# toverainc/willow-inference-server

Measured on NVIDIA H100. Metric: Whisper large-v2 realtime multiple (audio s / s), beam 5, 3.84 s utterance, higher is better.
Workload: dtype f16

## Files before the change

willow_inference_server_b200/csrc/encoder.cu:

```cuda
#include <algorithm>
#include <mutex>

#include "kernels.h"
#include "ptx.cuh"

namespace wisb {

void make_tmap_f16_2d(CUtensorMap* map, const void* ptr, long long cols, long long rows, long long ld, int box_cols,
                      int box_rows);

namespace {

constexpr int C1_FT = 64;
constexpr int C1_CT = 64;
template <int NM>
constexpr int c1_smem_bytes() { return (NM * (C1_FT + 2) + 3 * NM * (C1_CT + 1)) * 4; }

template <int NM>
__global__ void __launch_bounds__(256)
conv1_gelu_kernel(const float* __restrict__ mel, const __half* __restrict__ w, const float* __restrict__ bias,
                  __half* __restrict__ h1, int d) {
  constexpr int C1_K = 3 * NM;
  extern __shared__ float c1_smem[];
  float (*xm)[C1_FT + 2] = reinterpret_cast<float (*)[C1_FT + 2]>(c1_smem);
  float (*wt)[C1_CT + 1] = reinterpret_cast<float (*)[C1_CT + 1]>(c1_smem + NM * (C1_FT + 2));
  const int b = blockIdx.z;
  const int f0 = blockIdx.x * C1_FT;
  const int c0 = blockIdx.y * C1_CT;
  const int tid = threadIdx.x;
  const float* melb = mel + static_cast<long long>(b) * NM * N_FRAMES;
  for (int i = tid; i < NM * (C1_FT + 2); i += 256) {
    const int ci = i / (C1_FT + 2), fl = i % (C1_FT + 2);
    const int f = f0 + fl - 1;
    xm[ci][fl] = (f >= 0 && f < N_FRAMES) ? melb[ci * N_FRAMES + f] : 0.f;
  }
  for (int i = tid; i < C1_CT * C1_K; i += 256) {
    const int co = i / C1_K, kk = i % C1_K;
    wt[kk][co] = __half2float(w[static_cast<long long>(c0 + co) * C1_K + kk]);
  }
  __syncthreads();
  const int tc = tid % 16;
  const int tf = tid / 16;
  float acc[4][4];
#pragma unroll
  for (int i = 0; i < 4; ++i)
#pragma unroll
    for (int j = 0; j < 4; ++j) acc[i][j] = 0.f;
  for (int kk = 0; kk < C1_K; ++kk) {
    const int k = kk / NM, ci = kk - k * NM;
    float a[4], bb[4];
#pragma unroll
    for (int i = 0; i < 4; ++i) a[i] = xm[ci][tf * 4 + i + k];
#pragma unroll
    for (int j = 0; j < 4; ++j) bb[j] = wt[kk][tc * 4 + j];
#pragma unroll
    for (int i = 0; i < 4; ++i)
#pragma unroll
      for (int j = 0; j < 4; ++j) acc[i][j] = fmaf(a[i], bb[j], acc[i][j]);
  }
#pragma unroll
  for (int i = 0; i < 4; ++i) {
    const int f = f0 + tf * 4 + i;
    if (f >= N_FRAMES) continue;
    __half* o = h1 + (static_cast<long long>(b) * H1_ROWS + 1 + f) * d + c0 + tc * 4;
    __half2 v0 = __floats2half2_rn(gelu_erf(acc[i][0] + bias[c0 + tc * 4 + 0]), gelu_erf(acc[i][1] + bias[c0 + tc * 4 + 1]));
    __half2 v1 = __floats2half2_rn(gelu_erf(acc[i][2] + bias[c0 + tc * 4 + 2]), gelu_erf(acc[i][3] + bias[c0 + tc * 4 + 3]));
    uint2 u;
    u.x = *reinterpret_cast<uint32_t*>(&v0);
    u.y = *reinterpret_cast<uint32_t*>(&v1);
    *reinterpret_cast<uint2*>(o) = u;
  }
}

constexpr int LN_MAX_IT = 12;

__global__ void __launch_bounds__(256)
layernorm_f32_to_f16_kernel(const float* __restrict__ x, const float* __restrict__ g, const float* __restrict__ b,
                            __half* __restrict__ y, int rows, int d) {
  pdl_launch_dependents();
  pdl_wait();
  const int row = blockIdx.x * 8 + (threadIdx.x >> 5);
  const int lane = threadIdx.x & 31;
  if (row >= rows) return;
  const int iters = d / 128;
  const float4* xr = reinterpret_cast<const float4*>(x + static_cast<long long>(row) * d);
  float4 v[LN_MAX_IT];
  float s = 0.f;
#pragma unroll
  for (int i = 0; i < LN_MAX_IT; ++i)
    if (i < iters) {
      v[i] = xr[i * 32 + lane];
      s += v[i].x + v[i].y + v[i].z + v[i].w;
    }
  const float mean = warp_sum(s) / d;
  float q = 0.f;
#pragma unroll
  for (int i = 0; i < LN_MAX_IT; ++i)
    if (i < iters) {
      const float a0 = v[i].x - mean, a1 = v[i].y - mean, a2 = v[i].z - mean, a3 = v[i].w - mean;
      q += a0 * a0 + a1 * a1 + a2 * a2 + a3 * a3;
    }
  const float rstd = rsqrtf(warp_sum(q) / d + 1e-5f);
  const float4* g4 = reinterpret_cast<const float4*>(g);
  const float4* b4 = reinterpret_cast<const float4*>(b);
  uint2* yr = reinterpret_cast<uint2*>(y + static_cast<long long>(row) * d);
#pragma unroll
  for (int i = 0; i < LN_MAX_IT; ++i)
    if (i < iters) {
      const float4 gg = __ldg(g4 + i * 32 + lane), bb = __ldg(b4 + i * 32 + lane);
      __half2 h0 = __floats2half2_rn((v[i].x - mean) * rstd * gg.x + bb.x, (v[i].y - mean) * rstd * gg.y + bb.y);
      __half2 h1 = __floats2half2_rn((v[i].z - mean) * rstd * gg.z + bb.z, (v[i].w - mean) * rstd * gg.w + bb.w);
      uint2 u;
      u.x = *reinterpret_cast<uint32_t*>(&h0);
      u.y = *reinterpret_cast<uint32_t*>(&h1);
      yr[i * 32 + lane] = u;
    }
}

constexpr int AT_THREADS = 128;
constexpr int AT_BM = 64, AT_BN = 128;
constexpr int AT_NB = T_ENC_PAD / AT_BN;
constexpr int AT_TILE = 128 * 64 * 2;
constexpr int AT_Q_BYTES = AT_BM * 64 * 2;
constexpr int AT_SMEM = AT_Q_BYTES + 4 * AT_TILE  + 64  + 1024 ;

__device__ __forceinline__ uint32_t pack_half2(float a, float b) {
  __half2 h = __floats2half2_rn(a, b);
  return *reinterpret_cast<uint32_t*>(&h);
}

template <bool kVMN>
__global__ void __launch_bounds__(AT_THREADS, 3)
enc_attn_kernel(const __grid_constant__ CUtensorMap map_q, const __grid_constant__ CUtensorMap map_k,
                const __grid_constant__ CUtensorMap map_v, __half* __restrict__ ctx, int d, int H) {
  extern __shared__ uint8_t at_raw[];
  const uint32_t raw_addr = smem_u32(at_raw);
  const uint32_t base = (raw_addr + 1023u) & ~1023u;
  const uint32_t sQ = base;
  const uint32_t sK = base + AT_Q_BYTES;
  const uint32_t sV = sK + 2 * AT_TILE;
  const uint32_t bar0 = sV + 2 * AT_TILE;
  const uint32_t q_full = bar0;
  auto kv_full = [&](int s) { return bar0 + 8u * (1 + s); };

  const int tid = threadIdx.x, warp = tid >> 5, lane = tid & 31;
  const int qt = blockIdx.x, h = blockIdx.y, b = blockIdx.z;
  const int row0 = b * T_ENC_PAD + qt * AT_BM;

  if (tid == 0) {
    mbar_init(q_full, 1);
    mbar_init(kv_full(0), 1);
    mbar_init(kv_full(1), 1);
    fence_mbar_init();
    tma_prefetch_desc(&map_q);
    tma_prefetch_desc(&map_k);
    tma_prefetch_desc(&map_v);
  }
  __syncthreads();
  pdl_launch_dependents();
  pdl_wait();

  auto load_kv = [&](int j) {
    const int st = j & 1;
    mbar_arrive_expect_tx(kv_full(st), 2 * AT_TILE);
    tma_load_2d(sK + st * AT_TILE, &map_k, kv_full(st), d + h * HEAD_DIM, b * T_ENC_PAD + j * AT_BN);
    if (kVMN) {
      tma_load_2d(sV + st * AT_TILE, &map_v, kv_full(st), 2 * d + h * HEAD_DIM, b * T_ENC_PAD + j * AT_BN);
    } else {
      tma_load_2d(sV + st * AT_TILE, &map_v, kv_full(st), j * AT_BN, (b * H + h) * HEAD_DIM);
      tma_load_2d(sV + st * AT_TILE + AT_TILE / 2, &map_v, kv_full(st), j * AT_BN + 64, (b * H + h) * HEAD_DIM);
    }
  };
  if (tid == 0) {
    mbar_arrive_expect_tx(q_full, AT_Q_BYTES);
    tma_load_2d(sQ, &map_q, q_full, h * HEAD_DIM, row0);
    load_kv(0);
    load_kv(1);
  }

  const int cq = 2 * (lane & 3);
  const float c = 0.125f * 1.4426950408889634f;
  float m_run[2] = {-INFINITY, -INFINITY}, l_run[2] = {0.f, 0.f};
  float o[HEAD_DIM / 2];
#pragma unroll
  for (int i = 0; i < HEAD_DIM / 2; ++i) o[i] = 0.f;
  const uint64_t dq = make_desc_sw128(sQ, 1024);
  mbar_wait(q_full, 0);
#pragma unroll 1
  for (int j = 0; j < AT_NB; ++j) {
    const int st = j & 1;
    mbar_wait(kv_full(st), (j >> 1) & 1u);
    float s[AT_BN / 2];
    const uint64_t dk = make_desc_sw128(sK + st * AT_TILE, 1024);
    wgmma_fence();
#pragma unroll
    for (int k = 0; k < 4; ++k) wgmma_ss<AT_BN, 0, 0>(s, dq + 2u * k, dk + 2u * k, k != 0 ? 1u : 0u);
    wgmma_commit();
    wgmma_wait<0>();
    wgmma_reg_fence(s);
    const int kv0 = j * AT_BN;
    if (kv0 + AT_BN > T_ENC) {
#pragma unroll
      for (int i = 0; i < AT_BN / 2; ++i)
        if (kv0 + (i >> 2) * 8 + cq + (i & 1) >= T_ENC) s[i] = -INFINITY;
    }
    float alpha[2], mc[2];
#pragma unroll
    for (int hr = 0; hr < 2; ++hr) {
      float mx = -INFINITY;
#pragma unroll
      for (int nb = 0; nb < AT_BN / 8; ++nb) mx = fmaxf(mx, fmaxf(s[4 * nb + 2 * hr], s[4 * nb + 2 * hr + 1]));
      mx = fmaxf(mx, __shfl_xor_sync(0xffffffffu, mx, 1));
      mx = fmaxf(mx, __shfl_xor_sync(0xffffffffu, mx, 2));
      const float m_new = fmaxf(m_run[hr], mx);
      alpha[hr] = exp2f((m_run[hr] - m_new) * c);
      mc[hr] = m_new * c;
      m_run[hr] = m_new;
    }
    uint32_t pa[AT_BN / 16][4];
    float rs[2] = {0.f, 0.f};
#pragma unroll
    for (int kk = 0; kk < AT_BN / 16; ++kk) {
      float p[8];
#pragma unroll
      for (int i = 0; i < 8; ++i) {
        p[i] = exp2f(fmaf(s[8 * kk + i], c, -mc[(i >> 1) & 1]));
        rs[(i >> 1) & 1] += p[i];
      }
      pa[kk][0] = pack_half2(p[0], p[1]);
      pa[kk][1] = pack_half2(p[2], p[3]);
      pa[kk][2] = pack_half2(p[4], p[5]);
      pa[kk][3] = pack_half2(p[6], p[7]);
    }
#pragma unroll
    for (int hr = 0; hr < 2; ++hr) l_run[hr] = l_run[hr] * alpha[hr] + rs[hr];
#pragma unroll
    for (int i = 0; i < HEAD_DIM / 2; ++i) o[i] *= alpha[(i >> 1) & 1];
    wgmma_fence();
#pragma unroll
    for (int kk = 0; kk < AT_BN / 16; ++kk) {
      uint64_t dv;
      if (kVMN)
        dv = make_desc_sw128(sV + st * AT_TILE + kk * 2048, 1024);
      else
        dv = make_desc_sw128(sV + st * AT_TILE + (kk >> 2) * (AT_TILE / 2), 1024) + 2u * (kk & 3);
      wgmma_rs<HEAD_DIM, kVMN ? 1 : 0>(o, pa[kk], dv, 1u);
    }
    wgmma_commit();
    wgmma_wait<0>();
    wgmma_reg_fence(o);
    __syncthreads();
    if (tid == 0 && j + 2 < AT_NB) load_kv(j + 2);
  }
#pragma unroll
  for (int hr = 0; hr < 2; ++hr) {
    l_run[hr] += __shfl_xor_sync(0xffffffffu, l_run[hr], 1);
    l_run[hr] += __shfl_xor_sync(0xffffffffu, l_run[hr], 2);
  }
  const float inv[2] = {1.0f / l_run[0], 1.0f / l_run[1]};
#pragma unroll
  for (int hr = 0; hr < 2; ++hr) {
    const int r = warp * 16 + (lane >> 2) + 8 * hr;
    __half* out = ctx + static_cast<long long>(row0 + r) * d + h * HEAD_DIM + cq;
#pragma unroll
    for (int nb = 0; nb < HEAD_DIM / 8; ++nb)
      *reinterpret_cast<uint32_t*>(out + nb * 8) = pack_half2(o[4 * nb + 2 * hr] * inv[hr], o[4 * nb + 2 * hr + 1] * inv[hr]);
  }
}

__global__ void __launch_bounds__(128)
enc_attn_ref_kernel(const __half* __restrict__ qkv, __half* __restrict__ ctx, int d) {
  const int b = blockIdx.z, h = blockIdx.y;
  const int t = blockIdx.x * 128 + threadIdx.x;
  const long long ld = 3LL * d;
  const __half* base = qkv + static_cast<long long>(b) * T_ENC_PAD * ld;
  float q[HEAD_DIM], acc[HEAD_DIM];
  for (int e = 0; e < HEAD_DIM; ++e) {
    q[e] = __half2float(base[t * ld + h * HEAD_DIM + e]);
    acc[e] = 0.f;
  }
  float m = -INFINITY, l = 0.f;
  for (int k = 0; k < T_ENC; ++k) {
    const __half* kr = base + k * ld + d + h * HEAD_DIM;
    float s = 0.f;
    for (int e = 0; e < HEAD_DIM; ++e) s = fmaf(q[e], __half2float(kr[e]), s);
    s *= 0.125f;
    const float mn = fmaxf(m, s);
    const float a = __expf(m - mn), p = __expf(s - mn);
    const __half* vr = base + k * ld + 2 * d + h * HEAD_DIM;
    for (int e = 0; e < HEAD_DIM; ++e) acc[e] = acc[e] * a + p * __half2float(vr[e]);
    l = l * a + p;
    m = mn;
  }
  __half* o = ctx + (static_cast<long long>(b) * T_ENC_PAD + t) * d + h * HEAD_DIM;
  for (int e = 0; e < HEAD_DIM; ++e) o[e] = __float2half_rn(acc[e] / l);
}

}

void conv1_gelu_run(const float* mel, const __half* w, const float* bias, __half* h1, int B, int d, int n_mels,
                    cudaStream_t stream) {
  WISB_REQUIRE(d % C1_CT == 0, "conv1: d_model must be a multiple of 64");
  WISB_REQUIRE(n_mels == 80 || n_mels == 128, "conv1: n_mels must be 80 or 128");
  static std::atomic<unsigned long long> once{0};
  once_per_device(once, [] {
    WISB_CUDA(cudaFuncSetAttribute(conv1_gelu_kernel<80>, cudaFuncAttributeMaxDynamicSharedMemorySize, c1_smem_bytes<80>()));
    WISB_CUDA(cudaFuncSetAttribute(conv1_gelu_kernel<128>, cudaFuncAttributeMaxDynamicSharedMemorySize, c1_smem_bytes<128>()));
  });
  dim3 grid(cdiv(N_FRAMES, C1_FT), d / C1_CT, B);
  if (n_mels == 80)
    conv1_gelu_kernel<80><<<grid, 256, c1_smem_bytes<80>(), stream>>>(mel, w, bias, h1, d);
  else
    conv1_gelu_kernel<128><<<grid, 256, c1_smem_bytes<128>(), stream>>>(mel, w, bias, h1, d);
  WISB_CUDA(cudaGetLastError());
}

void layernorm_f32_to_f16_run(const float* x, const float* g, const float* b, __half* y, int rows, int d,
                              cudaStream_t stream, bool pdl) {
  WISB_REQUIRE(d % 128 == 0 && d <= 128 * LN_MAX_IT, "layernorm: d_model must be a multiple of 128, <= 1536");
  cudaLaunchConfig_t cfg{};
  cfg.gridDim = dim3(cdiv(rows, 8));
  cfg.blockDim = dim3(256);
  cfg.stream = stream;
  cudaLaunchAttribute attr[1];
  attr[0].id = cudaLaunchAttributeProgrammaticStreamSerialization;
  attr[0].val.programmaticStreamSerializationAllowed = 1;
  cfg.attrs = attr;
  cfg.numAttrs = pdl ? 1 : 0;
  WISB_CUDA(cudaLaunchKernelEx(&cfg, layernorm_f32_to_f16_kernel, x, g, b, y, rows, d));
}

void enc_attn_plan(AttnPlan& p, const __half* qkv, const __half* vt, __half* ctx, int B, int d, int H, bool v_mn_major) {
  p.B = B;
  p.d = d;
  p.H = H;
  p.ctx = ctx;
  p.v_mn_major = v_mn_major;
  const long long rows = static_cast<long long>(B) * T_ENC_PAD;
  make_tmap_f16_2d(&p.map_q, qkv, 3LL * d, rows, 3LL * d, 64, AT_BM);
  make_tmap_f16_2d(&p.map_k, qkv, 3LL * d, rows, 3LL * d, 64, 128);
  if (v_mn_major)
    make_tmap_f16_2d(&p.map_v, qkv, 3LL * d, rows, 3LL * d, 64, 128);
  else
    make_tmap_f16_2d(&p.map_v, vt, T_ENC_PAD, static_cast<long long>(B) * H * HEAD_DIM, T_ENC_PAD, 64, 64);
}

void enc_attn_run(const AttnPlan& p, cudaStream_t stream) {
  static std::atomic<unsigned long long> once{0};
  once_per_device(once, [] {
    WISB_CUDA(cudaFuncSetAttribute(enc_attn_kernel<true>, cudaFuncAttributeMaxDynamicSharedMemorySize, AT_SMEM));
    WISB_CUDA(cudaFuncSetAttribute(enc_attn_kernel<false>, cudaFuncAttributeMaxDynamicSharedMemorySize, AT_SMEM));
  });
  dim3 grid(T_ENC_PAD / AT_BM, p.H, p.B);
  cudaLaunchConfig_t cfg{};
  cfg.gridDim = grid;
  cfg.blockDim = dim3(AT_THREADS);
  cfg.dynamicSmemBytes = AT_SMEM;
  cfg.stream = stream;
  cudaLaunchAttribute attr[1];
  attr[0].id = cudaLaunchAttributeProgrammaticStreamSerialization;
  attr[0].val.programmaticStreamSerializationAllowed = 1;
  cfg.attrs = attr;
  cfg.numAttrs = p.pdl ? 1 : 0;
  if (p.v_mn_major)
    WISB_CUDA(cudaLaunchKernelEx(&cfg, enc_attn_kernel<true>, p.map_q, p.map_k, p.map_v, p.ctx, p.d, p.H));
  else
    WISB_CUDA(cudaLaunchKernelEx(&cfg, enc_attn_kernel<false>, p.map_q, p.map_k, p.map_v, p.ctx, p.d, p.H));
}

void enc_attn_ref_run(const __half* qkv, __half* ctx, int B, int d, int H, cudaStream_t stream) {
  dim3 grid(T_ENC_PAD / 128, H, B);
  enc_attn_ref_kernel<<<grid, 128, 0, stream>>>(qkv, ctx, d);
  WISB_CUDA(cudaGetLastError());
}

__global__ void __launch_bounds__(256) f32_to_f16_kernel(const float* __restrict__ x, __half* __restrict__ y, size_t n) {
  for (size_t i = blockIdx.x * 256ull + threadIdx.x; i < n; i += static_cast<size_t>(gridDim.x) * 256)
    y[i] = __float2half_rn(x[i]);
}

void f32_to_f16_run(const float* x, __half* y, size_t n, cudaStream_t stream) {
  const int grid = static_cast<int>(std::min<size_t>((n + 255) / 256, 8192));
  f32_to_f16_kernel<<<grid, 256, 0, stream>>>(x, y, n);
  WISB_CUDA(cudaGetLastError());
}

}
```

willow_inference_server_b200/csrc/kernels.h:

```cpp
#pragma once
#include "common.cuh"

namespace wisb {

enum EpiMode : int {
  EPI_F16 = 0,
  EPI_F16_GELU = 1,
  EPI_RESID_F32 = 2,
  EPI_CONV2 = 3,
  EPI_CROSSKV = 4,
  EPI_F32 = 5,
  EPI_QKV_VT = 6,
  EPI_DEC_QKV = 7,
};

struct GemmEpi {
  int mode = EPI_F16;
  const float* bias = nullptr;
  void* out = nullptr;
  long long ldo = 0;
  int m_valid = 0;
  int n_valid = 0;
  const float* pos = nullptr;
  void* aux = nullptr;
  void* aux2 = nullptr;
  int d_model = 0, n_heads = 0, batch = 0;
  int batch_off = 0;
  int kv_swizzle = 0;
  const int* row_slot = nullptr;
  const int* row_pos = nullptr;
  int t_cap = 0;
  long long split_stride = 0;
  const int* m_dyn = nullptr;
};

struct GemmPlan {
  CUtensorMap map_a, map_b;
  int M = 0, N = 0, K = 0, BN = 128, grid = 0, a_wrap = 0, mcast = 0, k_splits = 1, pdl = 0;
  GemmEpi epi;
};

void gemm_plan(GemmPlan& p, const __half* a, long long lda, const __half* w, int M, int N, int K, const GemmEpi& epi,
               int num_sms, int force_bn = 0, int a_wrap = 0, int k_splits = 1);
void gemm_run(const GemmPlan& p, cudaStream_t stream);
void gemm_ref_run(const __half* a, long long lda, const __half* w, float* c, int M, int N, int K, cudaStream_t stream);

void make_tmap_f16_2d(CUtensorMap* map, const void* ptr, long long cols, long long rows, long long ld, int box_cols,
                      int box_rows);

size_t logmel_table_floats();
void logmel_init_tables(float* tables_dev, int n_mels, cudaStream_t stream);
void logmel_run(const void* pcm, int pcm_is_s16, const long long* offsets_dev, const int* n_samples_dev, int B,
                int n_mels, const float* tables_dev, float* mel, unsigned* max_ws , cudaStream_t stream);

void conv1_gelu_run(const float* mel, const __half* w , const float* bias, __half* h1, int B, int d,
                    int n_mels, cudaStream_t stream);
void layernorm_f32_to_f16_run(const float* x, const float* g, const float* b, __half* y, int rows, int d,
                              cudaStream_t stream, bool pdl = false);
struct AttnPlan {
  CUtensorMap map_q, map_k, map_v;
  int B = 0, d = 0, H = 0;
  bool v_mn_major = true;
  bool pdl = false;
  __half* ctx = nullptr;
};
void enc_attn_plan(AttnPlan& p, const __half* qkv, const __half* vt, __half* ctx, int B, int d, int H, bool v_mn_major);
void enc_attn_run(const AttnPlan& p, cudaStream_t stream);
void enc_attn_ref_run(const __half* qkv, __half* ctx, int B, int d, int H, cudaStream_t stream);
void f32_to_f16_run(const float* x, __half* y, size_t n, cudaStream_t stream);

}
```

willow_inference_server_b200/csrc/ptx.cuh:

```cuda
#pragma once
#include <cuda.h>
#include <cuda_fp16.h>
#include <cuda_runtime.h>
#include <stdint.h>

namespace wisb {

__device__ __forceinline__ uint32_t smem_u32(const void* p) {
  return static_cast<uint32_t>(__cvta_generic_to_shared(p));
}

__device__ __forceinline__ bool elect_one() {
  uint32_t pred = 0;
  asm volatile(
      "{\n\t.reg .pred p;\n\t"
      "elect.sync _|p, 0xffffffff;\n\t"
      "selp.u32 %0, 1, 0, p;\n\t}"
      : "=r"(pred));
  return pred != 0;
}

__device__ __forceinline__ void mbar_init(uint32_t bar, uint32_t count) {
  asm volatile("mbarrier.init.shared::cta.b64 [%0], %1;" ::"r"(bar), "r"(count) : "memory");
}
__device__ __forceinline__ void fence_mbar_init() {
  asm volatile("fence.mbarrier_init.release.cluster;" ::: "memory");
}
__device__ __forceinline__ void fence_proxy_async_smem() {
  asm volatile("fence.proxy.async.shared::cta;" ::: "memory");
}
__device__ __forceinline__ void mbar_arrive_expect_tx(uint32_t bar, uint32_t bytes) {
  asm volatile("mbarrier.arrive.expect_tx.shared::cta.b64 _, [%0], %1;" ::"r"(bar), "r"(bytes) : "memory");
}
__device__ __forceinline__ void mbar_expect_tx(uint32_t bar, uint32_t bytes) {
  asm volatile("mbarrier.expect_tx.relaxed.cta.shared::cta.b64 [%0], %1;" ::"r"(bar), "r"(bytes) : "memory");
}
__device__ __forceinline__ void pdl_launch_dependents() { asm volatile("griddepcontrol.launch_dependents;" ::: "memory"); }
__device__ __forceinline__ void pdl_wait() { asm volatile("griddepcontrol.wait;" ::: "memory"); }
__device__ __forceinline__ void mbar_arrive(uint32_t bar) {
  asm volatile("mbarrier.arrive.shared::cta.b64 _, [%0];" ::"r"(bar) : "memory");
}
__device__ __forceinline__ void mbar_arrive_cluster(uint32_t bar, uint32_t cta) {
  asm volatile(
      "{\n\t.reg .b32 ra;\n\t"
      "mapa.shared::cluster.u32 ra, %0, %1;\n\t"
      "mbarrier.arrive.shared::cluster.b64 _, [ra];\n\t}" ::"r"(bar), "r"(cta)
      : "memory");
}
__device__ __forceinline__ bool mbar_try_wait(uint32_t bar, uint32_t parity) {
  uint32_t done;
  asm volatile(
      "{\n\t.reg .pred p;\n\t"
      "mbarrier.try_wait.parity.shared::cta.b64 p, [%1], %2;\n\t"
      "selp.u32 %0, 1, 0, p;\n\t}"
      : "=r"(done)
      : "r"(bar), "r"(parity)
      : "memory");
  return done != 0;
}
__device__ __forceinline__ void mbar_wait(uint32_t bar, uint32_t parity) {
  while (!mbar_try_wait(bar, parity)) {
  }
}

__device__ __forceinline__ void tma_prefetch_desc(const CUtensorMap* m) {
  asm volatile("prefetch.tensormap [%0];" ::"l"(reinterpret_cast<uint64_t>(m)) : "memory");
}
__device__ __forceinline__ void tma_load_2d(uint32_t dst, const CUtensorMap* m, uint32_t bar, int c0, int c1) {
  asm volatile(
      "cp.async.bulk.tensor.2d.shared::cluster.global.tile.mbarrier::complete_tx::bytes [%0], [%1, {%3, %4}], [%2];"
      ::"r"(dst), "l"(reinterpret_cast<uint64_t>(m)), "r"(bar), "r"(c0), "r"(c1)
      : "memory");
}
__device__ __forceinline__ void tma_load_2d_hint(uint32_t dst, const CUtensorMap* m, uint32_t bar, int c0, int c1, uint64_t pol) {
  asm volatile(
      "cp.async.bulk.tensor.2d.shared::cluster.global.tile.mbarrier::complete_tx::bytes.L2::cache_hint [%0], [%1, {%3, %4}], [%2], %5;"
      ::"r"(dst), "l"(reinterpret_cast<uint64_t>(m)), "r"(bar), "r"(c0), "r"(c1), "l"(pol)
      : "memory");
}
__device__ __forceinline__ void tma_load_3d(uint32_t dst, const CUtensorMap* m, uint32_t bar, int c0, int c1, int c2) {
  asm volatile(
      "cp.async.bulk.tensor.3d.shared::cluster.global.tile.mbarrier::complete_tx::bytes [%0], [%1, {%3, %4, %5}], [%2];"
      ::"r"(dst), "l"(reinterpret_cast<uint64_t>(m)), "r"(bar), "r"(c0), "r"(c1), "r"(c2)
      : "memory");
}
__device__ __forceinline__ void tma_load_2d_mcast(uint32_t dst, const CUtensorMap* m, uint32_t bar, int c0, int c1, uint16_t mask) {
  asm volatile(
      "cp.async.bulk.tensor.2d.shared::cluster.global.mbarrier::complete_tx::bytes.multicast::cluster [%0], [%1, {%4, %5}], [%2], %3;"
      ::"r"(dst), "l"(reinterpret_cast<uint64_t>(m)), "r"(bar), "h"(mask), "r"(c0), "r"(c1)
      : "memory");
}
__device__ __forceinline__ uint32_t cluster_ctarank() {
  uint32_t r;
  asm volatile("mov.u32 %0, %%cluster_ctarank;" : "=r"(r));
  return r;
}
__device__ __forceinline__ void cluster_sync_all() {
  asm volatile("barrier.cluster.arrive.release.aligned;\n\tbarrier.cluster.wait.acquire.aligned;" ::: "memory");
}
__device__ __forceinline__ void bulk_load_1d(uint32_t dst, const void* src, uint32_t bytes, uint32_t bar) {
  asm volatile("cp.async.bulk.shared::cluster.global.mbarrier::complete_tx::bytes [%0], [%1], %2, [%3];" ::"r"(dst),
               "l"(reinterpret_cast<uint64_t>(src)), "r"(bytes), "r"(bar)
               : "memory");
}

__device__ __forceinline__ uint64_t l2_policy_evict_first() {
  uint64_t pol;
  asm volatile("createpolicy.fractional.L2::evict_first.b64 %0, 1.0;" : "=l"(pol));
  return pol;
}
__device__ __forceinline__ void bulk_load_1d_hint(uint32_t dst, const void* src, uint32_t bytes, uint32_t bar, uint64_t pol) {
  asm volatile("cp.async.bulk.shared::cluster.global.mbarrier::complete_tx::bytes.L2::cache_hint [%0], [%1], %2, [%3], %4;" ::"r"(dst),
               "l"(reinterpret_cast<uint64_t>(src)), "r"(bytes), "r"(bar), "l"(pol)
               : "memory");
}

template <int N>
__device__ __forceinline__ void setmaxnreg_inc() { asm volatile("setmaxnreg.inc.sync.aligned.u32 %0;" ::"n"(N)); }
template <int N>
__device__ __forceinline__ void setmaxnreg_dec() { asm volatile("setmaxnreg.dec.sync.aligned.u32 %0;" ::"n"(N)); }
__device__ __forceinline__ void wgmma_fence() { asm volatile("wgmma.fence.sync.aligned;" ::: "memory"); }
__device__ __forceinline__ void wgmma_commit() { asm volatile("wgmma.commit_group.sync.aligned;" ::: "memory"); }
template <int N>
__device__ __forceinline__ void wgmma_wait() { asm volatile("wgmma.wait_group.sync.aligned %0;" ::"n"(N) : "memory"); }
template <int N>
__device__ __forceinline__ void wgmma_reg_fence(float (&d)[N]) {
#pragma unroll
  for (int i = 0; i < N; ++i) asm volatile("" : "+f"(d[i])::"memory");
}

template <int N, int TA, int TB>
__device__ __forceinline__ void wgmma_ss(float (&d)[N / 2], uint64_t desc_a, uint64_t desc_b, uint32_t scale_d);
template <int N, int TB>
__device__ __forceinline__ void wgmma_rs(float (&d)[N / 2], const uint32_t (&a)[4], uint64_t desc_b, uint32_t scale_d);

template <>
__device__ __forceinline__ void wgmma_ss<8, 0, 0>(float (&d)[4], uint64_t desc_a, uint64_t desc_b, uint32_t scale_d) {
  asm volatile(
      "{\n\t.reg .pred p;\n\t"
      "setp.ne.b32 p, %6, 0;\n\t"
      "wgmma.mma_async.sync.aligned.m64n8k16.f32.f16.f16 {%0, %1, %2, %3}, %4, %5, p, 1, 1, 0, 0;\n\t}"
      : "+f"(d[0]), "+f"(d[1]), "+f"(d[2]), "+f"(d[3])
      : "l"(desc_a), "l"(desc_b), "r"(scale_d));
}
template <>
__device__ __forceinline__ void wgmma_ss<8, 1, 0>(float (&d)[4], uint64_t desc_a, uint64_t desc_b, uint32_t scale_d) {
  asm volatile(
      "{\n\t.reg .pred p;\n\t"
      "setp.ne.b32 p, %6, 0;\n\t"
      "wgmma.mma_async.sync.aligned.m64n8k16.f32.f16.f16 {%0, %1, %2, %3}, %4, %5, p, 1, 1, 1, 0;\n\t}"
      : "+f"(d[0]), "+f"(d[1]), "+f"(d[2]), "+f"(d[3])
      : "l"(desc_a), "l"(desc_b), "r"(scale_d));
}
template <>
__device__ __forceinline__ void wgmma_ss<64, 0, 0>(float (&d)[32], uint64_t desc_a, uint64_t desc_b, uint32_t scale_d) {
  asm volatile(
      "{\n\t.reg .pred p;\n\t"
      "setp.ne.b32 p, %34, 0;\n\t"
      "wgmma.mma_async.sync.aligned.m64n64k16.f32.f16.f16 {%0, %1, %2, %3, %4, %5, %6, %7, %8, %9, %10, %11, %12, %13, %14, %15, %16, %17, %18, %19, %20, %21, %22, %23, %24, %25, %26, %27, %28, %29, %30, %31}, %32, %33, p, 1, 1, 0, 0;\n\t}"
      : "+f"(d[0]), "+f"(d[1]), "+f"(d[2]), "+f"(d[3]), "+f"(d[4]), "+f"(d[5]), "+f"(d[6]), "+f"(d[7]), "+f"(d[8]), "+f"(d[9]), "+f"(d[10]), "+f"(d[11]), "+f"(d[12]), "+f"(d[13]), "+f"(d[14]), "+f"(d[15]), "+f"(d[16]), "+f"(d[17]), "+f"(d[18]), "+f"(d[19]), "+f"(d[20]), "+f"(d[21]), "+f"(d[22]), "+f"(d[23]), "+f"(d[24]), "+f"(d[25]), "+f"(d[26]), "+f"(d[27]), "+f"(d[28]), "+f"(d[29]), "+f"(d[30]), "+f"(d[31])
      : "l"(desc_a), "l"(desc_b), "r"(scale_d));
}
template <>
__device__ __forceinline__ void wgmma_ss<128, 0, 0>(float (&d)[64], uint64_t desc_a, uint64_t desc_b, uint32_t scale_d) {
  asm volatile(
      "{\n\t.reg .pred p;\n\t"
      "setp.ne.b32 p, %66, 0;\n\t"
      "wgmma.mma_async.sync.aligned.m64n128k16.f32.f16.f16 {%0, %1, %2, %3, %4, %5, %6, %7, %8, %9, %10, %11, %12, %13, %14, %15, %16, %17, %18, %19, %20, %21, %22, %23, %24, %25, %26, %27, %28, %29, %30, %31, %32, %33, %34, %35, %36, %37, %38, %39, %40, %41, %42, %43, %44, %45, %46, %47, %48, %49, %50, %51, %52, %53, %54, %55, %56, %57, %58, %59, %60, %61, %62, %63}, %64, %65, p, 1, 1, 0, 0;\n\t}"
      : "+f"(d[0]), "+f"(d[1]), "+f"(d[2]), "+f"(d[3]), "+f"(d[4]), "+f"(d[5]), "+f"(d[6]), "+f"(d[7]), "+f"(d[8]), "+f"(d[9]), "+f"(d[10]), "+f"(d[11]), "+f"(d[12]), "+f"(d[13]), "+f"(d[14]), "+f"(d[15]), "+f"(d[16]), "+f"(d[17]), "+f"(d[18]), "+f"(d[19]), "+f"(d[20]), "+f"(d[21]), "+f"(d[22]), "+f"(d[23]), "+f"(d[24]), "+f"(d[25]), "+f"(d[26]), "+f"(d[27]), "+f"(d[28]), "+f"(d[29]), "+f"(d[30]), "+f"(d[31]), "+f"(d[32]), "+f"(d[33]), "+f"(d[34]), "+f"(d[35]), "+f"(d[36]), "+f"(d[37]), "+f"(d[38]), "+f"(d[39]), "+f"(d[40]), "+f"(d[41]), "+f"(d[42]), "+f"(d[43]), "+f"(d[44]), "+f"(d[45]), "+f"(d[46]), "+f"(d[47]), "+f"(d[48]), "+f"(d[49]), "+f"(d[50]), "+f"(d[51]), "+f"(d[52]), "+f"(d[53]), "+f"(d[54]), "+f"(d[55]), "+f"(d[56]), "+f"(d[57]), "+f"(d[58]), "+f"(d[59]), "+f"(d[60]), "+f"(d[61]), "+f"(d[62]), "+f"(d[63])
      : "l"(desc_a), "l"(desc_b), "r"(scale_d));
}
template <>
__device__ __forceinline__ void wgmma_ss<160, 0, 0>(float (&d)[80], uint64_t desc_a, uint64_t desc_b, uint32_t scale_d) {
  asm volatile(
      "{\n\t.reg .pred p;\n\t"
      "setp.ne.b32 p, %82, 0;\n\t"
      "wgmma.mma_async.sync.aligned.m64n160k16.f32.f16.f16 {%0, %1, %2, %3, %4, %5, %6, %7, %8, %9, %10, %11, %12, %13, %14, %15, %16, %17, %18, %19, %20, %21, %22, %23, %24, %25, %26, %27, %28, %29, %30, %31, %32, %33, %34, %35, %36, %37, %38, %39, %40, %41, %42, %43, %44, %45, %46, %47, %48, %49, %50, %51, %52, %53, %54, %55, %56, %57, %58, %59, %60, %61, %62, %63, %64, %65, %66, %67, %68, %69, %70, %71, %72, %73, %74, %75, %76, %77, %78, %79}, %80, %81, p, 1, 1, 0, 0;\n\t}"
      : "+f"(d[0]), "+f"(d[1]), "+f"(d[2]), "+f"(d[3]), "+f"(d[4]), "+f"(d[5]), "+f"(d[6]), "+f"(d[7]), "+f"(d[8]), "+f"(d[9]), "+f"(d[10]), "+f"(d[11]), "+f"(d[12]), "+f"(d[13]), "+f"(d[14]), "+f"(d[15]), "+f"(d[16]), "+f"(d[17]), "+f"(d[18]), "+f"(d[19]), "+f"(d[20]), "+f"(d[21]), "+f"(d[22]), "+f"(d[23]), "+f"(d[24]), "+f"(d[25]), "+f"(d[26]), "+f"(d[27]), "+f"(d[28]), "+f"(d[29]), "+f"(d[30]), "+f"(d[31]), "+f"(d[32]), "+f"(d[33]), "+f"(d[34]), "+f"(d[35]), "+f"(d[36]), "+f"(d[37]), "+f"(d[38]), "+f"(d[39]), "+f"(d[40]), "+f"(d[41]), "+f"(d[42]), "+f"(d[43]), "+f"(d[44]), "+f"(d[45]), "+f"(d[46]), "+f"(d[47]), "+f"(d[48]), "+f"(d[49]), "+f"(d[50]), "+f"(d[51]), "+f"(d[52]), "+f"(d[53]), "+f"(d[54]), "+f"(d[55]), "+f"(d[56]), "+f"(d[57]), "+f"(d[58]), "+f"(d[59]), "+f"(d[60]), "+f"(d[61]), "+f"(d[62]), "+f"(d[63]), "+f"(d[64]), "+f"(d[65]), "+f"(d[66]), "+f"(d[67]), "+f"(d[68]), "+f"(d[69]), "+f"(d[70]), "+f"(d[71]), "+f"(d[72]), "+f"(d[73]), "+f"(d[74]), "+f"(d[75]), "+f"(d[76]), "+f"(d[77]), "+f"(d[78]), "+f"(d[79])
      : "l"(desc_a), "l"(desc_b), "r"(scale_d));
}
template <>
__device__ __forceinline__ void wgmma_ss<256, 0, 0>(float (&d)[128], uint64_t desc_a, uint64_t desc_b, uint32_t scale_d) {
  asm volatile(
      "{\n\t.reg .pred p;\n\t"
      "setp.ne.b32 p, %130, 0;\n\t"
      "wgmma.mma_async.sync.aligned.m64n256k16.f32.f16.f16 {%0, %1, %2, %3, %4, %5, %6, %7, %8, %9, %10, %11, %12, %13, %14, %15, %16, %17, %18, %19, %20, %21, %22, %23, %24, %25, %26, %27, %28, %29, %30, %31, %32, %33, %34, %35, %36, %37, %38, %39, %40, %41, %42, %43, %44, %45, %46, %47, %48, %49, %50, %51, %52, %53, %54, %55, %56, %57, %58, %59, %60, %61, %62, %63, %64, %65, %66, %67, %68, %69, %70, %71, %72, %73, %74, %75, %76, %77, %78, %79, %80, %81, %82, %83, %84, %85, %86, %87, %88, %89, %90, %91, %92, %93, %94, %95, %96, %97, %98, %99, %100, %101, %102, %103, %104, %105, %106, %107, %108, %109, %110, %111, %112, %113, %114, %115, %116, %117, %118, %119, %120, %121, %122, %123, %124, %125, %126, %127}, %128, %129, p, 1, 1, 0, 0;\n\t}"
      : "+f"(d[0]), "+f"(d[1]), "+f"(d[2]), "+f"(d[3]), "+f"(d[4]), "+f"(d[5]), "+f"(d[6]), "+f"(d[7]), "+f"(d[8]), "+f"(d[9]), "+f"(d[10]), "+f"(d[11]), "+f"(d[12]), "+f"(d[13]), "+f"(d[14]), "+f"(d[15]), "+f"(d[16]), "+f"(d[17]), "+f"(d[18]), "+f"(d[19]), "+f"(d[20]), "+f"(d[21]), "+f"(d[22]), "+f"(d[23]), "+f"(d[24]), "+f"(d[25]), "+f"(d[26]), "+f"(d[27]), "+f"(d[28]), "+f"(d[29]), "+f"(d[30]), "+f"(d[31]), "+f"(d[32]), "+f"(d[33]), "+f"(d[34]), "+f"(d[35]), "+f"(d[36]), "+f"(d[37]), "+f"(d[38]), "+f"(d[39]), "+f"(d[40]), "+f"(d[41]), "+f"(d[42]), "+f"(d[43]), "+f"(d[44]), "+f"(d[45]), "+f"(d[46]), "+f"(d[47]), "+f"(d[48]), "+f"(d[49]), "+f"(d[50]), "+f"(d[51]), "+f"(d[52]), "+f"(d[53]), "+f"(d[54]), "+f"(d[55]), "+f"(d[56]), "+f"(d[57]), "+f"(d[58]), "+f"(d[59]), "+f"(d[60]), "+f"(d[61]), "+f"(d[62]), "+f"(d[63]), "+f"(d[64]), "+f"(d[65]), "+f"(d[66]), "+f"(d[67]), "+f"(d[68]), "+f"(d[69]), "+f"(d[70]), "+f"(d[71]), "+f"(d[72]), "+f"(d[73]), "+f"(d[74]), "+f"(d[75]), "+f"(d[76]), "+f"(d[77]), "+f"(d[78]), "+f"(d[79]), "+f"(d[80]), "+f"(d[81]), "+f"(d[82]), "+f"(d[83]), "+f"(d[84]), "+f"(d[85]), "+f"(d[86]), "+f"(d[87]), "+f"(d[88]), "+f"(d[89]), "+f"(d[90]), "+f"(d[91]), "+f"(d[92]), "+f"(d[93]), "+f"(d[94]), "+f"(d[95]), "+f"(d[96]), "+f"(d[97]), "+f"(d[98]), "+f"(d[99]), "+f"(d[100]), "+f"(d[101]), "+f"(d[102]), "+f"(d[103]), "+f"(d[104]), "+f"(d[105]), "+f"(d[106]), "+f"(d[107]), "+f"(d[108]), "+f"(d[109]), "+f"(d[110]), "+f"(d[111]), "+f"(d[112]), "+f"(d[113]), "+f"(d[114]), "+f"(d[115]), "+f"(d[116]), "+f"(d[117]), "+f"(d[118]), "+f"(d[119]), "+f"(d[120]), "+f"(d[121]), "+f"(d[122]), "+f"(d[123]), "+f"(d[124]), "+f"(d[125]), "+f"(d[126]), "+f"(d[127])
      : "l"(desc_a), "l"(desc_b), "r"(scale_d));
}
template <>
__device__ __forceinline__ void wgmma_rs<64, 0>(float (&d)[32], const uint32_t (&a)[4], uint64_t desc_b, uint32_t scale_d) {
  asm volatile(
      "{\n\t.reg .pred p;\n\t"
      "setp.ne.b32 p, %37, 0;\n\t"
      "wgmma.mma_async.sync.aligned.m64n64k16.f32.f16.f16 {%0, %1, %2, %3, %4, %5, %6, %7, %8, %9, %10, %11, %12, %13, %14, %15, %16, %17, %18, %19, %20, %21, %22, %23, %24, %25, %26, %27, %28, %29, %30, %31}, {%32, %33, %34, %35}, %36, p, 1, 1, 0;\n\t}"
      : "+f"(d[0]), "+f"(d[1]), "+f"(d[2]), "+f"(d[3]), "+f"(d[4]), "+f"(d[5]), "+f"(d[6]), "+f"(d[7]), "+f"(d[8]), "+f"(d[9]), "+f"(d[10]), "+f"(d[11]), "+f"(d[12]), "+f"(d[13]), "+f"(d[14]), "+f"(d[15]), "+f"(d[16]), "+f"(d[17]), "+f"(d[18]), "+f"(d[19]), "+f"(d[20]), "+f"(d[21]), "+f"(d[22]), "+f"(d[23]), "+f"(d[24]), "+f"(d[25]), "+f"(d[26]), "+f"(d[27]), "+f"(d[28]), "+f"(d[29]), "+f"(d[30]), "+f"(d[31])
      : "r"(a[0]), "r"(a[1]), "r"(a[2]), "r"(a[3]), "l"(desc_b), "r"(scale_d));
}
template <>
__device__ __forceinline__ void wgmma_rs<64, 1>(float (&d)[32], const uint32_t (&a)[4], uint64_t desc_b, uint32_t scale_d) {
  asm volatile(
      "{\n\t.reg .pred p;\n\t"
      "setp.ne.b32 p, %37, 0;\n\t"
      "wgmma.mma_async.sync.aligned.m64n64k16.f32.f16.f16 {%0, %1, %2, %3, %4, %5, %6, %7, %8, %9, %10, %11, %12, %13, %14, %15, %16, %17, %18, %19, %20, %21, %22, %23, %24, %25, %26, %27, %28, %29, %30, %31}, {%32, %33, %34, %35}, %36, p, 1, 1, 1;\n\t}"
      : "+f"(d[0]), "+f"(d[1]), "+f"(d[2]), "+f"(d[3]), "+f"(d[4]), "+f"(d[5]), "+f"(d[6]), "+f"(d[7]), "+f"(d[8]), "+f"(d[9]), "+f"(d[10]), "+f"(d[11]), "+f"(d[12]), "+f"(d[13]), "+f"(d[14]), "+f"(d[15]), "+f"(d[16]), "+f"(d[17]), "+f"(d[18]), "+f"(d[19]), "+f"(d[20]), "+f"(d[21]), "+f"(d[22]), "+f"(d[23]), "+f"(d[24]), "+f"(d[25]), "+f"(d[26]), "+f"(d[27]), "+f"(d[28]), "+f"(d[29]), "+f"(d[30]), "+f"(d[31])
      : "r"(a[0]), "r"(a[1]), "r"(a[2]), "r"(a[3]), "l"(desc_b), "r"(scale_d));
}

__device__ __forceinline__ void ldmatrix_x4(uint32_t addr, uint32_t (&r)[4]) {
  asm volatile("ldmatrix.sync.aligned.m8n8.x4.shared.b16 {%0, %1, %2, %3}, [%4];"
               : "=r"(r[0]), "=r"(r[1]), "=r"(r[2]), "=r"(r[3])
               : "r"(addr)
               : "memory");
}
__device__ __forceinline__ void ldmatrix_x4_trans(uint32_t addr, uint32_t (&r)[4]) {
  asm volatile("ldmatrix.sync.aligned.m8n8.x4.trans.shared.b16 {%0, %1, %2, %3}, [%4];"
               : "=r"(r[0]), "=r"(r[1]), "=r"(r[2]), "=r"(r[3])
               : "r"(addr)
               : "memory");
}
__device__ __forceinline__ void mma_m16n8k16(float (&c)[4], const uint32_t (&a)[4], uint32_t b0, uint32_t b1) {
  asm volatile(
      "mma.sync.aligned.m16n8k16.row.col.f32.f16.f16.f32 {%0, %1, %2, %3}, {%4, %5, %6, %7}, {%8, %9}, {%0, %1, %2, %3};"
      : "+f"(c[0]), "+f"(c[1]), "+f"(c[2]), "+f"(c[3])
      : "r"(a[0]), "r"(a[1]), "r"(a[2]), "r"(a[3]), "r"(b0), "r"(b1));
}

__device__ __forceinline__ uint64_t make_desc_sw128(uint32_t smem_addr, uint32_t sbo_bytes) {
  uint64_t d = 0;
  d |= static_cast<uint64_t>((smem_addr & 0x3FFFF) >> 4);
  d |= static_cast<uint64_t>(1) << 16;
  d |= static_cast<uint64_t>(sbo_bytes >> 4) << 32;
  d |= static_cast<uint64_t>(1) << 62;
  return d;
}

}
```

Baseline: 132.1.

## Warp-specialize persistent encoder attention with producer warp and pingpong consumers

Rewrites the encoder flash-attention kernel as a persistent, warp-specialized design: one producer warp issues TMA loads into a 4-stage K/V ring with full/empty mbarriers, and two consumer warpgroups each handle 64 query rows of a 128-row tile. The consumers alternate wgmma issue through named barriers and overlap the next QK^T with the current PV product, removing the per-iteration __syncthreads and serialized wait. It also switches to ex2.approx.ftz and rebalances registers with setmaxnreg. Cost: one CTA per SM with more shared memory, and more complex synchronization that could deadlock or load-imbalance.

```diff
diff --git a/willow_inference_server_b200/csrc/encoder.cu b/willow_inference_server_b200/csrc/encoder.cu
--- a/willow_inference_server_b200/csrc/encoder.cu
+++ b/willow_inference_server_b200/csrc/encoder.cu
@@ -117,40 +117,61 @@
     }
 }
 
-constexpr int AT_THREADS = 128;
-constexpr int AT_BM = 64, AT_BN = 128;
+constexpr int AT_CONSUMERS = 256;
+constexpr int AT_THREADS = AT_CONSUMERS + 128;
+constexpr int AT_WM = 64;
+constexpr int AT_BM = 2 * AT_WM;
+constexpr int AT_QT = T_ENC_PAD / AT_BM;
+constexpr int AT_BN = 128;
 constexpr int AT_NB = T_ENC_PAD / AT_BN;
+constexpr int AT_STAGES = 4;
 constexpr int AT_TILE = 128 * 64 * 2;
 constexpr int AT_Q_BYTES = AT_BM * 64 * 2;
-constexpr int AT_SMEM = AT_Q_BYTES + 4 * AT_TILE  + 64  + 1024 ;
+constexpr int AT_SMEM = 2 * AT_Q_BYTES + AT_STAGES * 2 * AT_TILE + 128  + 1024 ;
+constexpr int AT_BAR_TURN = 1;
 
 __device__ __forceinline__ uint32_t pack_half2(float a, float b) {
   __half2 h = __floats2half2_rn(a, b);
   return *reinterpret_cast<uint32_t*>(&h);
 }
+__device__ __forceinline__ float ex2_ftz(float x) {
+  float y;
+  asm("ex2.approx.ftz.f32 %0, %1;" : "=f"(y) : "f"(x));
+  return y;
+}
+__device__ __forceinline__ void wgmma_reg_fence_a(uint32_t (&a)[AT_BN / 16][4]) {
+#pragma unroll
+  for (int i = 0; i < AT_BN / 16; ++i)
+#pragma unroll
+    for (int k = 0; k < 4; ++k) asm volatile("" : "+r"(a[i][k])::"memory");
+}
 
 template <bool kVMN>
-__global__ void __launch_bounds__(AT_THREADS, 3)
+__global__ void __launch_bounds__(AT_THREADS, 1)
 enc_attn_kernel(const __grid_constant__ CUtensorMap map_q, const __grid_constant__ CUtensorMap map_k,
-                const __grid_constant__ CUtensorMap map_v, __half* __restrict__ ctx, int d, int H) {
+                const __grid_constant__ CUtensorMap map_v, __half* __restrict__ ctx, int d, int H, int items) {
   extern __shared__ uint8_t at_raw[];
   const uint32_t raw_addr = smem_u32(at_raw);
   const uint32_t base = (raw_addr + 1023u) & ~1023u;
-  const uint32_t sQ = base;
-  const uint32_t sK = base + AT_Q_BYTES;
-  const uint32_t sV = sK + 2 * AT_TILE;
-  const uint32_t bar0 = sV + 2 * AT_TILE;
-  const uint32_t q_full = bar0;
-  auto kv_full = [&](int s) { return bar0 + 8u * (1 + s); };
+  auto sQ = [&](int qb) { return base + qb * AT_Q_BYTES; };
+  auto sK = [&](int st) { return base + 2 * AT_Q_BYTES + st * 2 * AT_TILE; };
+  auto sV = [&](int st) { return sK(st) + AT_TILE; };
+  const uint32_t bar0 = base + 2 * AT_Q_BYTES + AT_STAGES * 2 * AT_TILE;
+  auto q_full = [&](int qb) { return bar0 + 8u * qb; };
+  auto q_empty = [&](int qb) { return bar0 + 8u * (2 + qb); };
+  auto kv_full = [&](int st) { return bar0 + 8u * (4 + st); };
+  auto kv_empty = [&](int st) { return bar0 + 8u * (4 + AT_STAGES + st); };
 
   const int tid = threadIdx.x, warp = tid >> 5, lane = tid & 31;
-  const int qt = blockIdx.x, h = blockIdx.y, b = blockIdx.z;
-  const int row0 = b * T_ENC_PAD + qt * AT_BM;
-
   if (tid == 0) {
-    mbar_init(q_full, 1);
-    mbar_init(kv_full(0), 1);
-    mbar_init(kv_full(1), 1);
+    for (int i = 0; i < 2; ++i) {
+      mbar_init(q_full(i), 1);
+      mbar_init(q_empty(i), 2);
+    }
+    for (int s = 0; s < AT_STAGES; ++s) {
+      mbar_init(kv_full(s), 1);
+      mbar_init(kv_empty(s), 2);
+    }
     fence_mbar_init();
     tma_prefetch_desc(&map_q);
     tma_prefetch_desc(&map_k);
@@ -160,112 +181,186 @@
   pdl_launch_dependents();
   pdl_wait();
 
-  auto load_kv = [&](int j) {
-    const int st = j & 1;
-    mbar_arrive_expect_tx(kv_full(st), 2 * AT_TILE);
-    tma_load_2d(sK + st * AT_TILE, &map_k, kv_full(st), d + h * HEAD_DIM, b * T_ENC_PAD + j * AT_BN);
-    if (kVMN) {
-      tma_load_2d(sV + st * AT_TILE, &map_v, kv_full(st), 2 * d + h * HEAD_DIM, b * T_ENC_PAD + j * AT_BN);
-    } else {
-      tma_load_2d(sV + st * AT_TILE, &map_v, kv_full(st), j * AT_BN, (b * H + h) * HEAD_DIM);
-      tma_load_2d(sV + st * AT_TILE + AT_TILE / 2, &map_v, kv_full(st), j * AT_BN + 64, (b * H + h) * HEAD_DIM);
-    }
-  };
-  if (tid == 0) {
-    mbar_arrive_expect_tx(q_full, AT_Q_BYTES);
-    tma_load_2d(sQ, &map_q, q_full, h * HEAD_DIM, row0);
-    load_kv(0);
-    load_kv(1);
-  }
+  auto item_qt = [&](int item) { return item % AT_QT; };
+  auto item_h = [&](int item) { return (item / AT_QT) % H; };
+  auto item_b = [&](int item) { return item / (AT_QT * H); };
+
+  if (warp >= AT_CONSUMERS / 32) {
+    setmaxnreg_dec<40>();
+    if (warp == AT_CONSUMERS / 32 && lane == 0) {
+      int n = 0;
+      int it = 0;
+      for (int item = blockIdx.x; item < items; item += gridDim.x, ++it) {
+        const int h = item_h(item), b = item_b(item);
+        const int qb = it & 1;
+        if (it >= 2) mbar_wait(q_empty(qb), ((it >> 1) - 1) & 1);
+        mbar_arrive_expect_tx(q_full(qb), AT_Q_BYTES);
+        const int row0 = b * T_ENC_PAD + item_qt(item) * AT_BM;
+        tma_load_2d(sQ(qb), &map_q, q_full(qb), h * HEAD_DIM, row0);
+        tma_load_2d(sQ(qb) + AT_Q_BYTES / 2, &map_q, q_full(qb), h * HEAD_DIM, row0 + AT_WM);
+        for (int j = 0; j < AT_NB; ++j, ++n) {
+          const int st = n % AT_STAGES;
+          if (n >= AT_STAGES) mbar_wait(kv_empty(st), ((n / AT_STAGES) - 1) & 1);
+          mbar_arrive_expect_tx(kv_full(st), 2 * AT_TILE);
+          tma_load_2d(sK(st), &map_k, kv_full(st), d + h * HEAD_DIM, b * T_ENC_PAD + j * AT_BN);
+          if (kVMN) {
+            tma_load_2d(sV(st), &map_v, kv_full(st), 2 * d + h * HEAD_DIM, b * T_ENC_PAD + j * AT_BN);
+          } else {
+            tma_load_2d(sV(st), &map_v, kv_full(st), j * AT_BN, (b * H + h) * HEAD_DIM);
+            tma_load_2d(sV(st) + AT_TILE / 2, &map_v, kv_full(st), j * AT_BN + 64, (b * H + h) * HEAD_DIM);
+          }
+        }
+      }
+    }
+    return;
+  }
+
+  setmaxnreg_inc<232>();
+  const int cw = warp >> 2;
+  const int wq = warp & 3;
+  const bool signaller = (tid & 127) == 0;
+  auto turn_begin = [&] { named_bar_sync<AT_CONSUMERS>(AT_BAR_TURN + cw); };
+  auto turn_end = [&] { named_bar_arrive<AT_CONSUMERS>(AT_BAR_TURN + (cw ^ 1)); };
+  if (cw == 1) turn_end();
 
   const int cq = 2 * (lane & 3);
   const float c = 0.125f * 1.4426950408889634f;
-  float m_run[2] = {-INFINITY, -INFINITY}, l_run[2] = {0.f, 0.f};
-  float o[HEAD_DIM / 2];
-#pragma unroll
-  for (int i = 0; i < HEAD_DIM / 2; ++i) o[i] = 0.f;
-  const uint64_t dq = make_desc_sw128(sQ, 1024);
-  mbar_wait(q_full, 0);
-#pragma unroll 1
-  for (int j = 0; j < AT_NB; ++j) {
-    const int st = j & 1;
-    mbar_wait(kv_full(st), (j >> 1) & 1u);
-    float s[AT_BN / 2];
-    const uint64_t dk = make_desc_sw128(sK + st * AT_TILE, 1024);
-    wgmma_fence();
+  auto issue_qk = [&](float (&s)[AT_BN / 2], uint64_t dq, int st) {
+    const uint64_t dk = make_desc_sw128(sK(st), 1024);
 #pragma unroll
     for (int k = 0; k < 4; ++k) wgmma_ss<AT_BN, 0, 0>(s, dq + 2u * k, dk + 2u * k, k != 0 ? 1u : 0u);
     wgmma_commit();
-    wgmma_wait<0>();
-    wgmma_reg_fence(s);
-    const int kv0 = j * AT_BN;
-    if (kv0 + AT_BN > T_ENC) {
-#pragma unroll
-      for (int i = 0; i < AT_BN / 2; ++i)
-        if (kv0 + (i >> 2) * 8 + cq + (i & 1) >= T_ENC) s[i] = -INFINITY;
-    }
-    float alpha[2], mc[2];
-#pragma unroll
-    for (int hr = 0; hr < 2; ++hr) {
-      float mx = -INFINITY;
-#pragma unroll
-      for (int nb = 0; nb < AT_BN / 8; ++nb) mx = fmaxf(mx, fmaxf(s[4 * nb + 2 * hr], s[4 * nb + 2 * hr + 1]));
-      mx = fmaxf(mx, __shfl_xor_sync(0xffffffffu, mx, 1));
-      mx = fmaxf(mx, __shfl_xor_sync(0xffffffffu, mx, 2));
-      const float m_new = fmaxf(m_run[hr], mx);
-      alpha[hr] = exp2f((m_run[hr] - m_new) * c);
-      mc[hr] = m_new * c;
-      m_run[hr] = m_new;
-    }
-    uint32_t pa[AT_BN / 16][4];
-    float rs[2] = {0.f, 0.f};
-#pragma unroll
-    for (int kk = 0; kk < AT_BN / 16; ++kk) {
-      float p[8];
-#pragma unroll
-      for (int i = 0; i < 8; ++i) {
-        p[i] = exp2f(fmaf(s[8 * kk + i], c, -mc[(i >> 1) & 1]));
-        rs[(i >> 1) & 1] += p[i];
-      }
-      pa[kk][0] = pack_half2(p[0], p[1]);
-      pa[kk][1] = pack_half2(p[2], p[3]);
-      pa[kk][2] = pack_half2(p[4], p[5]);
-      pa[kk][3] = pack_half2(p[6], p[7]);
-    }
-#pragma unroll
-    for (int hr = 0; hr < 2; ++hr) l_run[hr] = l_run[hr] * alpha[hr] + rs[hr];
-#pragma unroll
-    for (int i = 0; i < HEAD_DIM / 2; ++i) o[i] *= alpha[(i >> 1) & 1];
-    wgmma_fence();
+  };
+  auto issue_pv = [&](float (&o)[HEAD_DIM / 2], const uint32_t (&pa)[AT_BN / 16][4], int st) {
 #pragma unroll
     for (int kk = 0; kk < AT_BN / 16; ++kk) {
       uint64_t dv;
       if (kVMN)
-        dv = make_desc_sw128(sV + st * AT_TILE + kk * 2048, 1024);
+        dv = make_desc_sw128(sV(st) + kk * 2048, 1024);
       else
-        dv = make_desc_sw128(sV + st * AT_TILE + (kk >> 2) * (AT_TILE / 2), 1024) + 2u * (kk & 3);
+        dv = make_desc_sw128(sV(st) + (kk >> 2) * (AT_TILE / 2), 1024) + 2u * (kk & 3);
       wgmma_rs<HEAD_DIM, kVMN ? 1 : 0>(o, pa[kk], dv, 1u);
     }
     wgmma_commit();
+  };
+  auto release = [&](int st) {
+    if (signaller) mbar_arrive(kv_empty(st));
+  };
+
+  int n = 0;
+  int it = 0;
+#pragma unroll 1
+  for (int item = blockIdx.x; item < items; item += gridDim.x, ++it) {
+    const int h = item_h(item), b = item_b(item);
+    const int qb = it & 1;
+    const int row0 = b * T_ENC_PAD + item_qt(item) * AT_BM + cw * AT_WM;
+    const uint64_t dq = make_desc_sw128(sQ(qb) + cw * (AT_Q_BYTES / 2), 1024);
+    float m_run[2] = {-INFINITY, -INFINITY}, l_run[2] = {0.f, 0.f};
+    float o[HEAD_DIM / 2];
+#pragma unroll
+    for (int i = 0; i < HEAD_DIM / 2; ++i) o[i] = 0.f;
+    float s[AT_BN / 2];
+    uint32_t pa[AT_BN / 16][4];
+    mbar_wait(q_full(qb), (it >> 1) & 1);
+
+    float alpha[2], rs[2];
+    auto softmax = [&](int j) {
+      const int kv0 = j * AT_BN;
+      if (kv0 + AT_BN > T_ENC) {
+#pragma unroll
+        for (int i = 0; i < AT_BN / 2; ++i)
+          if (kv0 + (i >> 2) * 8 + cq + (i & 1) >= T_ENC) s[i] = -INFINITY;
+      }
+      float mc[2];
+#pragma unroll
+      for (int hr = 0; hr < 2; ++hr) {
+        float mx = -INFINITY;
+#pragma unroll
+        for (int nb = 0; nb < AT_BN / 8; ++nb) mx = fmaxf(mx, fmaxf(s[4 * nb + 2 * hr], s[4 * nb + 2 * hr + 1]));
+        mx = fmaxf(mx, __shfl_xor_sync(0xffffffffu, mx, 1));
+        mx = fmaxf(mx, __shfl_xor_sync(0xffffffffu, mx, 2));
+        const float m_new = fmaxf(m_run[hr], mx);
+        alpha[hr] = ex2_ftz((m_run[hr] - m_new) * c);
+        mc[hr] = m_new * c;
+        m_run[hr] = m_new;
+      }
+      rs[0] = rs[1] = 0.f;
+#pragma unroll
+      for (int i = 0; i < AT_BN / 2; ++i) {
+        s[i] = ex2_ftz(fmaf(s[i], c, -mc[(i >> 1) & 1]));
+        rs[(i >> 1) & 1] += s[i];
+      }
+    };
+    auto rescale_pack = [&] {
+#pragma unroll
+      for (int hr = 0; hr < 2; ++hr) l_run[hr] = l_run[hr] * alpha[hr] + rs[hr];
+#pragma unroll
+      for (int i = 0; i < HEAD_DIM / 2; ++i) o[i] *= alpha[(i >> 1) & 1];
+#pragma unroll
+      for (int kk = 0; kk < AT_BN / 16; ++kk) {
+        pa[kk][0] = pack_half2(s[8 * kk + 0], s[8 * kk + 1]);
+        pa[kk][1] = pack_half2(s[8 * kk + 2], s[8 * kk + 3]);
+        pa[kk][2] = pack_half2(s[8 * kk + 4], s[8 * kk + 5]);
+        pa[kk][3] = pack_half2(s[8 * kk + 6], s[8 * kk + 7]);
+      }
+    };
+
+    int st = n % AT_STAGES;
+    mbar_wait(kv_full(st), (n / AT_STAGES) & 1);
+    turn_begin();
+    wgmma_fence();
+    issue_qk(s, dq, st);
+    turn_end();
+    wgmma_wait<0>();
+    wgmma_reg_fence(s);
+    softmax(0);
+    rescale_pack();
+#pragma unroll 1
+    for (int j = 1; j < AT_NB; ++j) {
+      const int st_pv = st;
+      ++n;
+      st = n % AT_STAGES;
+      mbar_wait(kv_full(st), (n / AT_STAGES) & 1);
+      turn_begin();
+      wgmma_fence();
+      issue_qk(s, dq, st);
+      issue_pv(o, pa, st_pv);
+      turn_end();
+      wgmma_wait<1>();
+      wgmma_reg_fence(s);
+      softmax(j);
+      wgmma_wait<0>();
+      wgmma_reg_fence(o);
+      wgmma_reg_fence_a(pa);
+      release(st_pv);
+      rescale_pack();
+    }
+    turn_begin();
+    wgmma_fence();
+    issue_pv(o, pa, st);
+    turn_end();
+    ++n;
     wgmma_wait<0>();
     wgmma_reg_fence(o);
-    __syncthreads();
-    if (tid == 0 && j + 2 < AT_NB) load_kv(j + 2);
-  }
-#pragma unroll
-  for (int hr = 0; hr < 2; ++hr) {
-    l_run[hr] += __shfl_xor_sync(0xffffffffu, l_run[hr], 1);
-    l_run[hr] += __shfl_xor_sync(0xffffffffu, l_run[hr], 2);
-  }
-  const float inv[2] = {1.0f / l_run[0], 1.0f / l_run[1]};
-#pragma unroll
-  for (int hr = 0; hr < 2; ++hr) {
-    const int r = warp * 16 + (lane >> 2) + 8 * hr;
-    __half* out = ctx + static_cast<long long>(row0 + r) * d + h * HEAD_DIM + cq;
-#pragma unroll
-    for (int nb = 0; nb < HEAD_DIM / 8; ++nb)
-      *reinterpret_cast<uint32_t*>(out + nb * 8) = pack_half2(o[4 * nb + 2 * hr] * inv[hr], o[4 * nb + 2 * hr + 1] * inv[hr]);
-  }
+    wgmma_reg_fence_a(pa);
+    release(st);
+    if (signaller) mbar_arrive(q_empty(qb));
+#pragma unroll
+    for (int hr = 0; hr < 2; ++hr) {
+      l_run[hr] += __shfl_xor_sync(0xffffffffu, l_run[hr], 1);
+      l_run[hr] += __shfl_xor_sync(0xffffffffu, l_run[hr], 2);
+    }
+    const float inv[2] = {1.0f / l_run[0], 1.0f / l_run[1]};
+#pragma unroll
+    for (int hr = 0; hr < 2; ++hr) {
+      const int r = wq * 16 + (lane >> 2) + 8 * hr;
+      __half* out = ctx + static_cast<long long>(row0 + r) * d + h * HEAD_DIM + cq;
+#pragma unroll
+      for (int nb = 0; nb < HEAD_DIM / 8; ++nb)
+        *reinterpret_cast<uint32_t*>(out + nb * 8) = pack_half2(o[4 * nb + 2 * hr] * inv[hr], o[4 * nb + 2 * hr + 1] * inv[hr]);
+    }
+  }
+  if (cw == 0) turn_begin();
 }
 
 __global__ void __launch_bounds__(128)
@@ -336,8 +431,13 @@
   p.H = H;
   p.ctx = ctx;
   p.v_mn_major = v_mn_major;
+  int dev = 0, sms = 0;
+  WISB_CUDA(cudaGetDevice(&dev));
+  WISB_CUDA(cudaDeviceGetAttribute(&sms, cudaDevAttrMultiProcessorCount, dev));
+  p.items = AT_QT * H * B;
+  p.grid = cdiv(p.items, cdiv(p.items, sms));
   const long long rows = static_cast<long long>(B) * T_ENC_PAD;
-  make_tmap_f16_2d(&p.map_q, qkv, 3LL * d, rows, 3LL * d, 64, AT_BM);
+  make_tmap_f16_2d(&p.map_q, qkv, 3LL * d, rows, 3LL * d, 64, AT_WM);
   make_tmap_f16_2d(&p.map_k, qkv, 3LL * d, rows, 3LL * d, 64, 128);
   if (v_mn_major)
     make_tmap_f16_2d(&p.map_v, qkv, 3LL * d, rows, 3LL * d, 64, 128);
@@ -351,9 +451,8 @@
     WISB_CUDA(cudaFuncSetAttribute(enc_attn_kernel<true>, cudaFuncAttributeMaxDynamicSharedMemorySize, AT_SMEM));
     WISB_CUDA(cudaFuncSetAttribute(enc_attn_kernel<false>, cudaFuncAttributeMaxDynamicSharedMemorySize, AT_SMEM));
   });
-  dim3 grid(T_ENC_PAD / AT_BM, p.H, p.B);
   cudaLaunchConfig_t cfg{};
-  cfg.gridDim = grid;
+  cfg.gridDim = dim3(p.grid);
   cfg.blockDim = dim3(AT_THREADS);
   cfg.dynamicSmemBytes = AT_SMEM;
   cfg.stream = stream;
@@ -363,9 +462,9 @@
   cfg.attrs = attr;
   cfg.numAttrs = p.pdl ? 1 : 0;
   if (p.v_mn_major)
-    WISB_CUDA(cudaLaunchKernelEx(&cfg, enc_attn_kernel<true>, p.map_q, p.map_k, p.map_v, p.ctx, p.d, p.H));
+    WISB_CUDA(cudaLaunchKernelEx(&cfg, enc_attn_kernel<true>, p.map_q, p.map_k, p.map_v, p.ctx, p.d, p.H, p.items));
   else
-    WISB_CUDA(cudaLaunchKernelEx(&cfg, enc_attn_kernel<false>, p.map_q, p.map_k, p.map_v, p.ctx, p.d, p.H));
+    WISB_CUDA(cudaLaunchKernelEx(&cfg, enc_attn_kernel<false>, p.map_q, p.map_k, p.map_v, p.ctx, p.d, p.H, p.items));
 }
 
 void enc_attn_ref_run(const __half* qkv, __half* ctx, int B, int d, int H, cudaStream_t stream) {
diff --git a/willow_inference_server_b200/csrc/kernels.h b/willow_inference_server_b200/csrc/kernels.h
--- a/willow_inference_server_b200/csrc/kernels.h
+++ b/willow_inference_server_b200/csrc/kernels.h
@@ -60,6 +60,7 @@
 struct AttnPlan {
   CUtensorMap map_q, map_k, map_v;
   int B = 0, d = 0, H = 0;
+  int items = 0, grid = 0;
   bool v_mn_major = true;
   bool pdl = false;
   __half* ctx = nullptr;
diff --git a/willow_inference_server_b200/csrc/ptx.cuh b/willow_inference_server_b200/csrc/ptx.cuh
--- a/willow_inference_server_b200/csrc/ptx.cuh
+++ b/willow_inference_server_b200/csrc/ptx.cuh
@@ -119,6 +119,10 @@
 __device__ __forceinline__ void setmaxnreg_inc() { asm volatile("setmaxnreg.inc.sync.aligned.u32 %0;" ::"n"(N)); }
 template <int N>
 __device__ __forceinline__ void setmaxnreg_dec() { asm volatile("setmaxnreg.dec.sync.aligned.u32 %0;" ::"n"(N)); }
+template <int N>
+__device__ __forceinline__ void named_bar_sync(int id) { asm volatile("bar.sync %0, %1;" ::"r"(id), "n"(N) : "memory"); }
+template <int N>
+__device__ __forceinline__ void named_bar_arrive(int id) { asm volatile("bar.arrive %0, %1;" ::"r"(id), "n"(N) : "memory"); }
 __device__ __forceinline__ void wgmma_fence() { asm volatile("wgmma.fence.sync.aligned;" ::: "memory"); }
 __device__ __forceinline__ void wgmma_commit() { asm volatile("wgmma.commit_group.sync.aligned;" ::: "memory"); }
 template <int N>
```

Result: no change. 132.3 (median of 6 runs) (+0.1%).
